# teasgen/speech_separation

Measured on AMD Instinct MI355X. Metric: mixtures/sec (2-spk, 4 s @ 8 kHz) DPTN-AV forward, higher is better.
Workload: dtype f32; 1 GPU; configs[2]: DPTN-AV (dptn_wav_av) forward, precomputed lip embeddings, batch=16 per GPU, T=32000, random-init weights (numpy seed 0); batch_per_gpu=16, samples=32000, parallelism=dp1 (batch shards, no data-path collective)

## Files before the change

### speech_separation_amd/csrc/attn_block.h

```cpp
#pragma once
#include "common.h"

constexpr int ATTN_BLOCK_MAX_LEN = 160;
size_t attn_block_lds_bytes(int nkb);
struct AttnFfnPrologue {
  const float* hc;
  const float* wf;
  const float* bf;
  const float* g2;
  const float* b2;
};
constexpr int ATTN_PACK_IN = 3 * 128 * 128, ATTN_PACK_OUT = 128 * 128, ATTN_PACK_FFN = 128 * 256;
constexpr int ATTN_PACK_FLOATS = ATTN_PACK_IN + ATTN_PACK_OUT + ATTN_PACK_FFN;
struct AttnPackSrc {
  const float* w_in;
  const float* w_o;
  const float* w_f;
};
constexpr int ATTN_PACK_MAX_PATHS = 32;
int attn_pack_launch(void* stream, const AttnPackSrc* src, int npaths, float* dst );
int attn_block_launch(void* stream, const float* x, const float* w_in, const float* b_in, const float* w_o, const float* b_o,
                      const float* gamma, const float* beta, float* y1, const SeqGeom& g, bool split = false,
                      const AttnFfnPrologue* pro = nullptr, const float* wpack = nullptr);

size_t attn_block2_lds_bytes(int nkb, bool pro);
int attn_block2_launch(void* stream, const float* x, const float* b_in, const float* b_o, const float* gamma, const float* beta,
                       float* y1, const SeqGeom& g, const AttnFfnPrologue* pro, const float* wpack);
```

### speech_separation_amd/csrc/attn_block2.hip

```cpp
#include <hip/hip_runtime.h>

#include "attn_block.h"
#include "vmem_asm.h"

namespace {

constexpr int N = 128, DH = 32;
constexpr int LDX = N + 4;
constexpr int LDHC = 256 + 4;
constexpr int OB_FLOATS = 4 * 4 * 64 * 4;

constexpr int kb_mfmas(int kb, int nkb) { return (kb > 0 ? 16 : 0) + (kb + 1 < nkb ? 16 : 0); }

DEV void ln_group_stats(f32x16& v, float& mu_w, float& m2_w) {
  f32x2 s0 = (f32x2){v[0], v[1]} + (f32x2){v[2], v[3]}, s1 = (f32x2){v[4], v[5]} + (f32x2){v[6], v[7]};
  s0 += (f32x2){v[8], v[9]};
  s1 += (f32x2){v[10], v[11]};
  s0 += (f32x2){v[12], v[13]};
  s1 += (f32x2){v[14], v[15]};
  const f32x2 s = s0 + s1;
  mu_w = half_sum(s.x + s.y) * (1.0f / 32);
  const f32x2 m2 = (f32x2){mu_w, mu_w};
  f32x2 q0 = (f32x2){0.f, 0.f}, q1 = (f32x2){0.f, 0.f};
#pragma unroll
  for (int r = 0; r < 16; r += 4) {
    const f32x2 d0 = (f32x2){v[r], v[r + 1]} - m2, d1 = (f32x2){v[r + 2], v[r + 3]} - m2;
    v[r] = d0.x; v[r + 1] = d0.y; v[r + 2] = d1.x; v[r + 3] = d1.y;
    q0 += d0 * d0;
    q1 += d1 * d1;
  }
  const f32x2 q = q0 + q1;
  m2_w = half_sum(q.x + q.y);
}
DEV float ln_merge(const float4 a, const float4 b, float mu_w, float& delta) {
  const float mu = ((a.x + a.z) + (b.x + b.z)) * 0.25f;
  const float d0 = a.x - mu, d1 = a.z - mu, d2 = b.x - mu, d3 = b.z - mu;
  const float m2 = ((a.y + a.w) + (b.y + b.w)) + 32.0f * ((d0 * d0 + d1 * d1) + (d2 * d2 + d3 * d3));
  delta = mu_w - mu;
  return rsqrtf(m2 * (1.0f / N) + 1e-5f);
}

struct FfnPro2 {
  const float* hc;
  const float* wf;
  const float* bf;
  const float* g2;
  const float* b2;
};

#ifdef ATTN_STAMPS
__device__ unsigned long long g_ab2_stamps[16];
DEV unsigned long long ab_now() {
  unsigned long long t;
  asm volatile("s_memtime %0\n\ts_waitcnt lgkmcnt(0)" : "=s"(t) :: "memory");
  return t;
}
#define AB_DECL unsigned long long ab_t[12] = {0, 0, 0, 0, 0, 0, 0, 0, 0, 0, 0, 0}; unsigned long long ab_last = ab_now();
#define AB_MARK(i) { const unsigned long long ab_n = ab_now(); ab_t[i] += ab_n - ab_last; ab_last = ab_n; }
#define AB_KEEP(x) asm volatile("" :: "v"(x));
#define AB_END                                                                                      \
  if ((threadIdx.x & 63) == 0) {                                                                    \
    for (int ab_i = 0; ab_i < 12; ++ab_i) atomicAdd(&g_ab2_stamps[ab_i], ab_t[ab_i]);               \
    atomicAdd(&g_ab2_stamps[12], 1ull);                                                             \
  }
#else
#define AB_DECL
#define AB_MARK(i)
#define AB_KEEP(x)
#define AB_END
#endif

template <int NKB, bool PRO>
__global__ __launch_bounds__(256) void attn_block2_kernel(const float* __restrict__ x, const float* __restrict__ wp_in,
                                                          const float* __restrict__ b_in, const float* __restrict__ wp_o,
                                                          const float* __restrict__ b_o, const float* __restrict__ gamma,
                                                          const float* __restrict__ beta, float* __restrict__ y1, SeqGeom g,
                                                          float scale_log2e, FfnPro2 pro) {
  extern __shared__ __attribute__((aligned(16))) float smem[];
  float* Xs = smem;
  float* Hs = smem + NKB * 32 * LDX;
  float* Ob = Hs;
  float* Red = Hs + (PRO ? 2 * 32 * LDHC : OB_FLOATS);
  float* Cst = Red + 512;
  const int tid = threadIdx.x;
  const int h = __builtin_amdgcn_readfirstlane(tid >> 6);
  const int lane = tid & 63, c = lane & 31, hh = lane >> 5;
  const int seq = blockIdx.x, len = g.len;
  const int64_t tok0 = seq_token_base(g, seq);
  const int tstride = seq_token_stride(g);
  const unsigned rs_y = (unsigned)tstride * 512u;
  char* const ybase = reinterpret_cast<char*>(y1) + tok0 * 512;
  auto row_off = [&](int row, unsigned rstride, bool clamp) -> unsigned {
    if (clamp) row = row < len ? row : len - 1;
    return (unsigned)__umul24((unsigned)row, rstride);
  };
  const unsigned frag_col = (unsigned)(32 * h + 4 * hh);

  AB_DECL
  if (tid < (PRO ? 192 : 96)) {
    const int which = tid >> 5, q4 = tid & 31;
    const float* src = which == 0 ? b_o : which == 1 ? gamma : which == 2 ? beta : which == 3 ? pro.bf : which == 4 ? pro.g2 : pro.b2;
    *reinterpret_cast<float4*>(&Cst[which * 128 + 4 * q4]) = ldg4(src + 4 * q4);
  }
  auto cst16 = [&](int which, f32x16& d) {
#pragma unroll
    for (int j = 0; j < 4; ++j) {
      const float4 t = *reinterpret_cast<const float4*>(&Cst[which * 128 + frag_col + 8 * j]);
      d[4 * j + 0] = t.x; d[4 * j + 1] = t.y; d[4 * j + 2] = t.z; d[4 * j + 3] = t.w;
    }
  };
  auto red_put = [&](int par, float mu_w, float m2_w) {
    *reinterpret_cast<float2*>(&Red[par * 256 + (c * 4 + h) * 2]) = make_float2(mu_w, m2_w);
  };
  auto red_get = [&](int par, float mu_w, float& delta) {
    const float4 a = *reinterpret_cast<const float4*>(&Red[par * 256 + c * 8]), b = *reinterpret_cast<const float4*>(&Red[par * 256 + c * 8 + 4]);
    return ln_merge(a, b, mu_w, delta);
  };

  float wkf[64], wvf[64];
  auto fetch_wkv1 = [&](int m) {
    const float* wk = wp_in + ((1 * 4 + h) * 16 * 64 + lane) * 4;
    const float* wv = wp_in + ((2 * 4 + h) * 16 * 64 + lane) * 4;
    const float4 a = ldg4(wk + m * 256), b = ldg4(wv + m * 256);
    wkf[4 * m + 0] = a.x; wkf[4 * m + 1] = a.y; wkf[4 * m + 2] = a.z; wkf[4 * m + 3] = a.w;
    wvf[4 * m + 0] = b.x; wvf[4 * m + 1] = b.y; wvf[4 * m + 2] = b.z; wvf[4 * m + 3] = b.w;
  };
  auto fetch_wkv = [&]() {
#pragma unroll
    for (int m = 0; m < 16; ++m) fetch_wkv1(m);
  };
  if constexpr (PRO) {
    f32x4 wf4[32];
    const uint32_t lane16 = (uint32_t)lane * 16u;
    {
      const char* wb = reinterpret_cast<const char*>(pro.wf + h * 32 * 64 * 4);
      static_for<8>([&](auto MQ) {
        constexpr int mq = decltype(MQ)::value;
        ldg4_uncounted_a<0>(wf4[4 * mq + 0], wb + mq * 4096, lane16);
        ldg4_uncounted_a<1024>(wf4[4 * mq + 1], wb + mq * 4096, lane16);
        ldg4_uncounted_a<2048>(wf4[4 * mq + 2], wb + mq * 4096, lane16);
        ldg4_uncounted_a<3072>(wf4[4 * mq + 3], wb + mq * 4096, lane16);
      });
    }
    const uint32_t hs_lds = lds_addr(Hs);
    const char* const hbase = reinterpret_cast<const char*>(pro.hc) + tok0 * 1024;
    const uint32_t rs_h = (uint32_t)tstride * 1024u;
    constexpr bool TRI = NKB >= 4;
    auto hbuf_lds = [&](int b) -> uint32_t {
      if (TRI) return (b % 3) == 2 ? lds_addr(Xs) + (uint32_t)((NKB - 2) * 32 * LDX * 4) : hs_lds + (uint32_t)((b % 3) * 32 * LDHC * 4);
      return hs_lds + (uint32_t)((b & 1) * 32 * LDHC * 4);
    };
    auto hbuf = [&](int b) -> const float* { return TRI ? ((b % 3) == 2 ? Xs + (NKB - 2) * 32 * LDX : Hs + (b % 3) * 32 * LDHC) : Hs + (b & 1) * 32 * LDHC; };
    f32x4 res[2][4];
    auto issue_d1 = [&](auto RB, int i) {
      constexpr int rb = decltype(RB)::value;
      int row = rb * 32 + 8 * h + i;
      if (rb == NKB - 1) row = row < len ? row : len - 1;
      dma_part<false>(hbase + (uint32_t)row * rs_h, lane16, hbuf_lds(rb) + (uint32_t)((8 * h + i) * LDHC * 4));
    };
    auto issue_r1 = [&](auto RB, f32x4 (&rr)[4], int j) {
      constexpr int rb = decltype(RB)::value;
      const unsigned ro = row_off(rb * 32 + c, rs_y, rb == NKB - 1) + 4u * frag_col;
      switch (j) {
        case 0: ldg4_uncounted<0>(rr[0], ybase, ro); break;
        case 1: ldg4_uncounted<32>(rr[1], ybase, ro); break;
        case 2: ldg4_uncounted<64>(rr[2], ybase, ro); break;
        default: ldg4_uncounted<96>(rr[3], ybase, ro); break;
      }
    };
    auto issue_d = [&](auto RB) {
#pragma unroll
      for (int i = 0; i < 8; ++i) issue_d1(RB, i);
    };
    auto issue_r = [&](auto RB, f32x4 (&rr)[4]) {
#pragma unroll
      for (int j = 0; j < 4; ++j) issue_r1(RB, rr, j);
    };
    constexpr int AHEAD = TRI ? 2 : 1;
    issue_d(std::integral_constant<int, 0>{});
    issue_r(std::integral_constant<int, 0>{}, res[0]);
    constexpr int BEHIND_WF = 12;
    wait_vm_a16<BEHIND_WF>(wf4);
    wait_vm_a16<BEHIND_WF>(wf4 + 16);
    AB_MARK(0)
    f32x16 vprev = zero16();
    float mu_prev = 0.f;
    auto normalise_prev = [&](int pb) {
      float delta;
      const float rstd = red_get(pb & 1, mu_prev, delta);
      f32x16 g2c, b2c;
      cst16(4, g2c);
      cst16(5, b2c);
      const f32x2 d2 = (f32x2){delta, delta}, r2 = (f32x2){rstd, rstd};
      float* xw = &Xs[(pb * 32 + c) * LDX + frag_col];
#pragma unroll
      for (int j = 0; j < 4; ++j) {
        const f32x2 lo = ((f32x2){vprev[4 * j], vprev[4 * j + 1]} + d2) * r2 * (f32x2){g2c[4 * j], g2c[4 * j + 1]} + (f32x2){b2c[4 * j], b2c[4 * j + 1]};
        const f32x2 hi = ((f32x2){vprev[4 * j + 2], vprev[4 * j + 3]} + d2) * r2 * (f32x2){g2c[4 * j + 2], g2c[4 * j + 3]} +
                         (f32x2){b2c[4 * j + 2], b2c[4 * j + 3]};
        *reinterpret_cast<float4*>(xw + 8 * j) = make_float4(lo.x, lo.y, hi.x, hi.y);
      }
    };
    auto pro_block = [&](auto RB) {
      constexpr int rb = decltype(RB)::value;
      constexpr int KEEP = (AHEAD == 2 && rb >= 1 && rb + 1 < NKB) ? 8 : 0;
      wait_vm<KEEP>(res[rb & 1]);
      __syncthreads();
      AB_MARK(1)
      constexpr bool HAS_R = rb + 1 < NKB, HAS_D = rb + AHEAD < NKB && rb + AHEAD >= 2, HAS_D1 = rb == 0 && NKB > 1;
      constexpr int NREQ = rb == NKB - 1 ? 16 : 4 + (HAS_D1 ? 8 : 0) + (HAS_D ? 8 : 0);
      auto request = [&](int k) {
        if constexpr (rb == NKB - 1) {
          fetch_wkv1(k);
        } else if (k < 4) {
          if constexpr (HAS_R) issue_r1(std::integral_constant<int, HAS_R ? rb + 1 : 0>{}, res[(rb + 1) & 1], k);
        } else if (HAS_D1 && k < 12) {
          if constexpr (HAS_D1) issue_d1(std::integral_constant<int, 1>{}, k - 4);
        } else {
          if constexpr (HAS_D) issue_d1(std::integral_constant<int, HAS_D ? rb + AHEAD : 0>{}, k - (HAS_D1 ? 12 : 4));
        }
      };
      f32x16 a0 = zero16(), a1 = zero16();
      const float* ar = hbuf(rb) + c * LDHC + 4 * hh;
#pragma unroll
      for (int m0 = 0; m0 < 32; m0 += 8) {
        float4 af[8];
#pragma unroll
        for (int m = 0; m < 8; ++m) af[m] = *reinterpret_cast<const float4*>(ar + 8 * (m0 + m));
#pragma unroll
        for (int m = 0; m < 8; ++m) {
          a0 = mfma32(wf4[m0 + m][0], af[m].x, a0);
          a1 = mfma32(wf4[m0 + m][1], af[m].y, a1);
          a0 = mfma32(wf4[m0 + m][2], af[m].z, a0);
          a1 = mfma32(wf4[m0 + m][3], af[m].w, a1);
          constexpr int EVERY = NREQ > 12 ? 1 : 2;
          if ((m0 + m) % EVERY == EVERY - 1 && (m0 + m) / EVERY < NREQ && (m0 + m) < 24) {
            __builtin_amdgcn_sched_barrier(0);
            request((m0 + m) / EVERY);
            __builtin_amdgcn_sched_barrier(0);
          }
        }
// ... 9 lines not shown
      AB_KEEP(a0[15]) AB_KEEP(a1[15])
      AB_MARK(2)
      f32x16 bfc;
      cst16(3, bfc);
#pragma unroll
      for (int r = 0; r < 16; r += 2) {
        const f32x2 t = ((f32x2){a0[r], a0[r + 1]} + (f32x2){a1[r], a1[r + 1]}) + (f32x2){bfc[r], bfc[r + 1]} +
                        (f32x2){res[rb & 1][r >> 2][r & 3], res[rb & 1][r >> 2][(r & 3) + 1]};
        vprev[r] = t.x;
        vprev[r + 1] = t.y;
      }
      float m2_w;
      ln_group_stats(vprev, mu_prev, m2_w);
      red_put(rb & 1, mu_prev, m2_w);
      AB_MARK(3)
    };
    static_for<NKB>(pro_block);
    __syncthreads();
    normalise_prev(NKB - 1);
    AB_MARK(4)
  } else {
    constexpr int NLD = NKB * 4;
    float4 st[NLD];
#pragma unroll
    for (int i = 0; i < NLD; ++i) {
      const int row = i * 8 + (tid >> 5);
      st[i] = *reinterpret_cast<const float4*>(reinterpret_cast<const char*>(x) + tok0 * 512 + row_off(row, rs_y, i >= 4 * (NKB - 1)) +
                                               16u * (tid & 31));
    }
    fetch_wkv();
#pragma unroll
    for (int i = 0; i < NLD; ++i) *reinterpret_cast<float4*>(&Xs[(i * 8 + (tid >> 5)) * LDX + 4 * (tid & 31)]) = st[i];
  }
  __syncthreads();
  AB_MARK(5)

  float wqf[64];
  {
    const float* wq = wp_in + ((0 * 4 + h) * 16 * 64 + lane) * 4;
#pragma unroll
    for (int m = 0; m < 16; ++m) {
      const float4 a = ldg4(wq + m * 256);
      wqf[4 * m + 0] = a.x; wqf[4 * m + 1] = a.y; wqf[4 * m + 2] = a.z; wqf[4 * m + 3] = a.w;
    }
  }
  f32x16 kt[NKB], vv[NKB];
  {
    const float bv = b_in[2 * N + h * DH + c];
    float bk[16];
#pragma unroll
    for (int j = 0; j < 4; ++j) {
      const float4 t = ldg4(b_in + N + h * DH + 8 * j + 4 * hh);
      bk[4 * j + 0] = t.x; bk[4 * j + 1] = t.y; bk[4 * j + 2] = t.z; bk[4 * j + 3] = t.w;
    }
#pragma unroll
    for (int rb = 0; rb < NKB; ++rb) {
      const float* xr = &Xs[(rb * 32 + c) * LDX + 4 * hh];
      f32x16 ka = zero16(), va = zero16();
#pragma unroll
      for (int m0 = 0; m0 < 16; m0 += 8) {
        float4 xf[8];
#pragma unroll
        for (int m = 0; m < 8; ++m) xf[m] = *reinterpret_cast<const float4*>(xr + 8 * (m0 + m));
#pragma unroll
        for (int m = 0; m < 8; ++m) {
          const float xa[4] = {xf[m].x, xf[m].y, xf[m].z, xf[m].w};
#pragma unroll
          for (int t = 0; t < 4; ++t) {
            ka = mfma32(wkf[4 * (m0 + m) + t], xa[t], ka);
            va = mfma32(xa[t], wvf[4 * (m0 + m) + t], va);
          }
        }
      }
#pragma unroll
      for (int r = 0; r < 16; r += 2) {
        const f32x2 tk = (f32x2){ka[r], ka[r + 1]} + (f32x2){bk[r], bk[r + 1]}, tv = (f32x2){va[r], va[r + 1]} + (f32x2){bv, bv};
        kt[rb][r] = tk.x; kt[rb][r + 1] = tk.y;
        vv[rb][r] = tv.x; vv[rb][r + 1] = tv.y;
      }
#pragma unroll
      for (int r = 0; r < 16; ++r) asm volatile("" : "+a"(kt[rb][r]), "+a"(vv[rb][r]));
      __builtin_amdgcn_sched_barrier(0);
    }
  }

  AB_MARK(6)
#pragma unroll
  for (int i = 0; i < 64; ++i) asm volatile("" : "+a"(wqf[i]));
  float wo2[4][16];
#pragma unroll
  for (int hp = 0; hp < 4; ++hp) {
    const float* wr = wp_o + (((hp * 4 + h) * 4) * 64 + lane) * 4;
#pragma unroll
    for (int j = 0; j < 4; ++j) {
      const float4 t = ldg4(wr + j * 256);
      wo2[hp][4 * j + 0] = t.x; wo2[hp][4 * j + 1] = t.y; wo2[hp][4 * j + 2] = t.z; wo2[hp][4 * j + 3] = t.w;
    }
  }
  float qbias[16];
#pragma unroll
  for (int j = 0; j < 4; ++j) {
    const float4 t = ldg4(b_in + h * DH + 8 * j + 4 * hh);
    qbias[4 * j + 0] = t.x; qbias[4 * j + 1] = t.y; qbias[4 * j + 2] = t.z; qbias[4 * j + 3] = t.w;
  }

  auto q_tile_mfmas = [&](int qb, f32x16& q0, f32x16& q1) {
    const float* xr = &Xs[(qb * 32 + c) * LDX + 4 * hh];
#pragma unroll
    for (int m0 = 0; m0 < 16; m0 += 8) {
      float4 xf[8];
#pragma unroll
      for (int m = 0; m < 8; ++m) xf[m] = *reinterpret_cast<const float4*>(xr + 8 * (m0 + m));
#pragma unroll
      for (int m = 0; m < 8; ++m) {
        q0 = mfma32(wqf[4 * (m0 + m) + 0], xf[m].x, q0);
        q1 = mfma32(wqf[4 * (m0 + m) + 1], xf[m].y, q1);
// ... 140 lines not shown
    AB_MARK(9)
    __builtin_amdgcn_sched_barrier(0);
    if (qb + 1 < NKB) {
      qa = zero16();
      qb_ = zero16();
      q_tile_mfmas(qb + 1, qa, qb_);
    }
    {
      const float rstd = red_get(0, mu_w, delta);
      f32x16 gac, bec;
      cst16(1, gac);
      cst16(2, bec);
      const f32x2 d2 = (f32x2){delta, delta}, r2 = (f32x2){rstd, rstd};
      char* yw = ybase + row_off(qb * 32 + c, rs_y, true) + 4u * frag_col;
#pragma unroll
      for (int j = 0; j < 4; ++j) {
        const f32x2 lo = ((f32x2){v[4 * j], v[4 * j + 1]} + d2) * r2 * (f32x2){gac[4 * j], gac[4 * j + 1]} + (f32x2){bec[4 * j], bec[4 * j + 1]};
        const f32x2 hi = ((f32x2){v[4 * j + 2], v[4 * j + 3]} + d2) * r2 * (f32x2){gac[4 * j + 2], gac[4 * j + 3]} +
                         (f32x2){bec[4 * j + 2], bec[4 * j + 3]};
        *reinterpret_cast<float4*>(yw + 32 * j) = make_float4(lo.x, lo.y, hi.x, hi.y);
      }
    }
    if (qb + 1 < NKB) {
#pragma unroll
      for (int i = 0; i < 64; ++i) {
        __builtin_amdgcn_sched_group_barrier(0x008, 1, 0);
        __builtin_amdgcn_sched_group_barrier(0x1f6, 2, 0);
      }
    }
    __builtin_amdgcn_sched_barrier(0);
    AB_KEEP(qa[15]) AB_KEEP(qb_[15])
    AB_MARK(10)
  }
  AB_END
}

}

size_t attn_block2_lds_bytes(int nkb, bool pro) {
  return sizeof(float) * ((size_t)nkb * 32 * LDX + (pro ? 2 * 32 * LDHC : OB_FLOATS) + 512 + 6 * 128);
}

int attn_block2_launch(void* stream, const float* x, const float* b_in, const float* b_o, const float* gamma, const float* beta,
                       float* y1, const SeqGeom& g, const AttnFfnPrologue* pro, const float* wpack) {
  using Kern = void (*)(const float*, const float*, const float*, const float*, const float*, const float*, const float*, float*,
                        SeqGeom, float, FfnPro2);
  const int nkb = (g.len + 31) / 32;
  if (nkb < 1 || nkb > 5 || !wpack) return (int)hipErrorInvalidValue;
  const float scale_log2e = 1.4426950408889634f / sqrtf((float)DH);
  const int dev = current_hip_device();
  Kern kern;
  const bool p = pro != nullptr;
  switch (nkb) {
    case 1: kern = p ? attn_block2_kernel<1, true> : attn_block2_kernel<1, false>; break;
    case 2: kern = p ? attn_block2_kernel<2, true> : attn_block2_kernel<2, false>; break;
    case 3: kern = p ? attn_block2_kernel<3, true> : attn_block2_kernel<3, false>; break;
    case 4: kern = p ? attn_block2_kernel<4, true> : attn_block2_kernel<4, false>; break;
    default: kern = p ? attn_block2_kernel<5, true> : attn_block2_kernel<5, false>; break;
  }
  const size_t lds = attn_block2_lds_bytes(nkb, p);
  static PerDeviceOnce ready_all[2][6];
  PerDeviceOnce* ready = ready_all[p ? 1 : 0];
  if (!ready[nkb].done(dev)) {
    hipError_t e = hipFuncSetAttribute(reinterpret_cast<const void*>(kern), hipFuncAttributeMaxDynamicSharedMemorySize, (int)lds);
    if (e != hipSuccess) return (int)e;
    ready[nkb].set(dev);
  }
  FfnPro2 fp{};
  if (p) fp = FfnPro2{pro->hc, pro->wf, pro->bf, pro->g2, pro->b2};
  hipLaunchKernelGGL(kern, dim3(g.nseq), dim3(256), lds, static_cast<hipStream_t>(stream), x, wpack, b_in, wpack + ATTN_PACK_IN,
                     b_o, gamma, beta, y1, g, scale_log2e, fp);
  return (int)hipGetLastError();
}

#ifdef ATTN_STAMPS
extern "C" int dptnav_debug_attn2_stamps(unsigned long long* out, int reset) {
  if (reset) {
    unsigned long long z[16] = {0};
    return (int)hipMemcpyToSymbol(HIP_SYMBOL(g_ab2_stamps), z, sizeof(z));
  }
  if (hipDeviceSynchronize() != hipSuccess) return -1;
  return (int)hipMemcpyFromSymbol(out, HIP_SYMBOL(g_ab2_stamps), 16 * sizeof(unsigned long long));
}
#endif
```

### speech_separation_amd/csrc/dptnav.hip

```cpp
#include <hip/hip_runtime.h>

#include <cmath>
#include <cstdarg>
#include <cstdio>
#include <cstring>
#include <string>
#include <vector>

#include "../../include/dptnav.h"
#include "attention.h"
#include "attn_block.h"
#include "attn_block64.h"
#include "common.h"
#include "gemm_ws.h"
#include "headtail.h"
#include "lstm.h"
#include "lstm16.h"
#include "fcln.h"
#include "dgrad_t.h"
#include "dgrad_r.h"
#include "gemm_t.h"
#include "sisnr.h"
#include "train_tail.h"
#include "backward.h"
// ... 44 lines not shown

enum ProfCat { CAT_VIDEO = 0, CAT_ENCODER, CAT_QKV, CAT_ATTN, CAT_OUTPROJ, CAT_LSTM_PRE, CAT_LSTM, CAT_FFN,
               CAT_SEP, CAT_POST, CAT_DECODER, CAT_COUNT };
static const char* const kProfNames[CAT_COUNT] = {
    "video_linear", "encoder_fuse", "qkv_gemm", "attention", "outproj_ln_gemm", "lstm_pre_gemm",
    "lstm_recurrence", "ffn_ln_gemm", "sep_gemm", "postproc_gemm", "decoder_gather"};

struct ProfRec {
  int cat;
  hipEvent_t a, b;
};

struct dptnav_ctx {
  dptnav_config cfg;
  bool prof_on = false;
  bool opt_lstm_stamps = false;
  bool opt_overlap = true;
  bool opt_serialize = false;
  bool opt_lstm16 = true;
  int opt_fuse_pre128 = 1;
  bool fuse128_for(int B) const { return opt_fuse_pre128 == 2 || (opt_fuse_pre128 == 1 && B >= 12); }
  int opt_fcln = 1;
  bool opt_fuse_pre = true;
  bool opt_pack_whh = true;
  bool opt_pack_wih = true;
  bool opt_deterministic = false;
  int opt_lstm4 = 1;
  bool opt_split_bf16 = false;
  bool opt_fuse_attn = true;
  bool opt_gemm_t = true;
  bool opt_dgrad_r = true;
  bool opt_dgrad_t = true;
  bool opt_attn_v2 = true;
  bool opt_fold_tail = true;
  bool opt_wgrad_ride = true;
  bool opt_wgrad2 = true;
  bool opt_ln_tape = true;
  bool opt_fuse_ffn = true;
  int opt_lstm_diag = 0;
  int opt_inject_fail = 0;
  bool opt_debug_sync = false;
  bool opt_train_fuse_probe = false;
  int opt_dropout_ppm = 0;
  unsigned opt_dropout_seed = 0;
  DropCfg drop_cfg(int block, int path, bool train, int half = 0) const {
    DropCfg d{0u, 0u, 1.0f};
    if (!train || opt_dropout_ppm <= 0) return d;
    const double p = opt_dropout_ppm * 1e-6;
    d.seed = opt_dropout_seed ^ (0x9E3779B9u * (unsigned)(2 * block + path + 1)) ^ (0x7F4A7C15u * (unsigned)half);
    d.thresh = (unsigned)(p * 16777216.0);
    d.inv_keep = (float)(1.0 / (1.0 - p));
    return d;
  }
  static constexpr int NSTREAMS = 4;
  hipStream_t streams[NSTREAMS] = {nullptr, nullptr, nullptr, nullptr};
  hipEvent_t ev_fork = nullptr, ev_join[NSTREAMS] = {nullptr, nullptr, nullptr, nullptr}, ev_lstm[2] = {nullptr, nullptr};
  hipEvent_t ev_side[2][4] = {{nullptr, nullptr, nullptr, nullptr}, {nullptr, nullptr, nullptr, nullptr}};
  bool opt_wgrad_side = true;
  int opt_sub_batches = 0;
  int opt_lstm_inflight = 0;
  int opt_split_policy = 1;
  bool opt_lstm_chain = false;
  std::vector<hipEvent_t> ev_sub;
  int ensure_sub_events(int n) {
    while ((int)ev_sub.size() < n) {
      hipEvent_t e = nullptr;
// ... 560 lines not shown
  const int64_t ntiles = (M + BM - 1) / BM;
  const bool dptn = g.arch == 0;
  const float* lstm_in = dptn ? y1 : x_in;

  const bool fused = dptn && (!pb.train || c->opt_train_fuse_probe) && path_fusable<N>(c, path, B, S);
  if (fused && (chain & CHAIN_PRO) && c->pw[2 * block + path - 1].ndir != 2)
    return c->fail(DPTNAV_ERR_INVALID, "internal: FFN prologue needs both LSTM directions of the previous path");
  if (fused && N == 64) {
    ProfScope ps(c, CAT_ATTN, st);
    AttnFfnPrologue pro{};
    if (chain & CHAIN_PRO) {
      const PathWeights& pw = c->pw[2 * block + path - 1];
      pro = AttnFfnPrologue{hc, pw.ffn_w, pw.ffn_b, pw.ln2_w, pw.ln2_b};
    }
    const int rc = attn_block64_launch(st, x_in, w.in_w, w.in_b, w.out_w, w.out_b, w.ln1_w, w.ln1_b, y1, geom,
                                       (chain & CHAIN_PRO) ? &pro : nullptr);
    if (rc != 0) return c->fail(DPTNAV_ERR_HIP, "attention block (N = 64): %s", hipGetErrorString((hipError_t)rc));
  } else if (fused) {
    ProfScope ps(c, CAT_ATTN, st);
    AttnFfnPrologue pro{};
    if (chain & CHAIN_PRO) {
      const PathWeights& pw = c->pw[2 * block + path - 1];
      pro = AttnFfnPrologue{hc, pw.ffn_w, pw.ffn_b, pw.ln2_w, pw.ln2_b};
    }
    const float* wpack = nullptr;
    if (!c->opt_split_bf16) {
      float* pk = ws + pl.wpack + (size_t)(2 * block + path) * ATTN_PACK_FLOATS;
      if (!run.packed) {
        if (int rc = pack_attn_weights(c, st, 2 * block + path, 1, pk)) return rc;
      }
      wpack = pk;
      if (chain & CHAIN_PRO) pro.wf = pk - ATTN_PACK_FLOATS + ATTN_PACK_IN + ATTN_PACK_OUT;
    }
    const int rc = (c->opt_attn_v2 && !c->opt_split_bf16)
                       ? attn_block2_launch(st, x_in, w.in_b, w.out_b, w.ln1_w, w.ln1_b, y1, geom, (chain & CHAIN_PRO) ? &pro : nullptr, wpack)
                       : attn_block_launch(st, x_in, w.in_w, w.in_b, w.out_w, w.out_b, w.ln1_w, w.ln1_b, y1, geom, c->opt_split_bf16,
                                           (chain & CHAIN_PRO) ? &pro : nullptr, wpack);
    if (rc != 0) return c->fail(DPTNAV_ERR_HIP, "attention block: %s", hipGetErrorString((hipError_t)rc));
  } else if (chain & CHAIN_PRO) {
    return c->fail(DPTNAV_ERR_INVALID, "internal: FFN prologue requested for an unfused attention block");
  }
  if (dptn && !fused) {
    int done = 0;
    if constexpr (N == 128) {
      if (pb.train && c->opt_gemm_t) {
        if (int rc = inject_failure(c, "qkv gemm")) return rc;
        if (run.slot + 1 > QUEUE_SLOTS) return c->fail(DPTNAV_ERR_INVALID, "qkv gemm: ticket counters exhausted");
        float* wp = ws + pl.winp + (run.packed_inw ? (size_t)(2 * block + path) * 3 * N * N : 0);
        if (!run.packed_inw)
          if (int rc = pack_inw(c, st, 2 * block + path, 1, wp)) return rc;
        GemmTArgs ga;
        ga.A = x_in; ga.Wpacked = wp; ga.bias = w.in_b; ga.out = qkv; ga.M = M; ga.nout = 3 * N;
        unsigned* const queue = run.take_queue(1);
        ga.queue = c->opt_deterministic ? nullptr : queue;
        ProfScope ps(c, CAT_QKV, st);
        const int rc = gemm_t_launch(st, ga, c->num_cus);
        if (rc == 0) done = 1;
        else if (rc == (int)hipErrorInvalidValue) { (void)hipGetLastError(); run.slot -= 1; }
        else return c->fail(DPTNAV_ERR_HIP, "qkv gemm: %s", hipGetErrorString((hipError_t)rc));
      }
    }
    if (!done) {
      ALoadDense al{x_in, M, N, BM};
      EpiBiasStore ep{qkv, w.in_b, M, 3 * N, BM, 3 * N};
      if (int rc = launch_gemm<N, 3, WR, WC>(c, run, CAT_QKV, "qkv gemm", w.in_w, ntiles, 1, al, ep)) return rc;
    }
  }
  if (dptn && !fused)
// ... 1856 lines not shown
  return DPTNAV_OK;
}

int dptnav_dropout_mask(dptnav_handle h, int block, int path, int B, int S, float* mask, void* stream) {
  if (!h || !mask) return DPTNAV_ERR_INVALID;
  const SeqGeom geom = make_geom(path, B, S, h->cfg.chunk_size);
  hipLaunchKernelGGL(dropout_mask_kernel, dim3(geom.nseq, h->cfg.num_heads), dim3(256), 0, (hipStream_t)stream, mask, geom,
                     h->cfg.num_heads, h->drop_cfg(block, path, true));
  LAUNCH_CHECK(h, "dropout mask");
  return DPTNAV_OK;
}

int dptnav_set_option(dptnav_handle h, const char* key, int value) {
  if (!h || !key) return DPTNAV_ERR_INVALID;
  const std::string k(key);
  if (k == "lstm_stamps") h->opt_lstm_stamps = value != 0;
  else if (k == "dropout_ppm" && value >= 0 && value < 1000000) h->opt_dropout_ppm = value;
  else if (k == "dropout_seed") h->opt_dropout_seed = (unsigned)value;
  else if (k == "overlap") h->opt_overlap = value != 0;
  else if (k == "serialize") h->opt_serialize = value != 0;
  else if (k == "deterministic") h->opt_deterministic = value != 0;
  else if (k == "pack_wih") h->opt_pack_wih = value != 0;
  else if (k == "fuse_pre") h->opt_fuse_pre = value != 0;
  else if (k == "fcln" && value >= 0 && value <= 2) h->opt_fcln = value;
  else if (k == "fuse_pre128" && value >= 0 && value <= 2) h->opt_fuse_pre128 = value;
  else if (k == "pack_whh") h->opt_pack_whh = value != 0;
  else if (k == "lstm16") h->opt_lstm16 = value != 0;
  else if (k == "lstm4") {
    if (value < 0 || value > 2) return h->fail(DPTNAV_ERR_INVALID, "lstm4: 0, 1 or 2");
    h->opt_lstm4 = (int)value;
  }
  else if (k == "fuse_attn") h->opt_fuse_attn = value != 0;
  else if (k == "attn_v2") h->opt_attn_v2 = value != 0;
  else if (k == "dgrad_t") h->opt_dgrad_t = value != 0;
  else if (k == "dgrad_r") h->opt_dgrad_r = value != 0;
  else if (k == "gemm_t") h->opt_gemm_t = value != 0;
  else if (k == "fuse_ffn") h->opt_fuse_ffn = value != 0;
  else if (k == "wgrad2") h->opt_wgrad2 = value != 0;
  else if (k == "ln_tape") h->opt_ln_tape = value != 0;
  else if (k == "fold_tail") h->opt_fold_tail = value != 0;
  else if (k == "wgrad_ride") h->opt_wgrad_ride = value != 0;
  else if (k == "wgrad_side") h->opt_wgrad_side = value != 0;
  else if (k == "sub_batches" && value >= 0 && value <= MAX_SUB) h->opt_sub_batches = value;
  else if (k == "lstm_inflight" && value >= 0 && value <= MAX_SUB) h->opt_lstm_inflight = value;
  else if (k == "split_policy" && (value == 0 || value == 1)) h->opt_split_policy = value;
  else if (k == "lstm_chain") h->opt_lstm_chain = value != 0;
  else if (k == "split_bf16") h->opt_split_bf16 = value != 0;
  else if (k == "train_overlap") h->opt_train_overlap = value != 0;
  else if (k == "lstm_diag") h->opt_lstm_diag = (int)value;
  else if (k == "inject_fail") h->opt_inject_fail = value;
  else if (k == "debug_sync") h->opt_debug_sync = value != 0;
  else if (k == "train_fuse_probe") h->opt_train_fuse_probe = value != 0;
  else return h->fail(DPTNAV_ERR_INVALID, "unknown option '%s'", key);
  return DPTNAV_OK;
}

int dptnav_profile_enable(dptnav_handle h, int on) {
  if (!h) return DPTNAV_ERR_INVALID;
  h->prof_on = on != 0;
  return DPTNAV_OK;
}
int dptnav_profile_collect(dptnav_handle h) {
  if (!h) return DPTNAV_ERR_INVALID;
  for (ProfRec& r : h->prof_pending) {
    float ms = 0.f;
    hipError_t e = hipEventSynchronize(r.b);
// ... 50 lines not shown
```

### speech_separation_amd/csrc/vmem_asm.h

```cpp
#pragma once
#include "common.h"

DEV uint32_t lds_addr(const void* p) { return (uint32_t)(uintptr_t)(const __attribute__((address_space(3))) void*)p; }

template <bool HALF>
DEV void dma_part(const void* sbase, uint32_t voff, uint32_t lds_base) {
  if constexpr (!HALF) {
    asm volatile("s_mov_b32 m0, %0\n\ts_nop 4\n\tglobal_load_lds_dwordx4 %1, %2" ::"s"(lds_base), "v"(voff), "s"(sbase) : "memory", "m0");
  } else {
    uint32_t saved;
    asm volatile("s_mov_b32 m0, %1\n\ts_mov_b32 %0, exec_hi\n\ts_mov_b32 exec_hi, 0\n\ts_nop 4\n\tglobal_load_lds_dwordx4 %2, %3\n\ts_mov_b32 exec_hi, %0"
                 : "=&s"(saved)
                 : "s"(lds_base), "v"(voff), "s"(sbase)
                 : "memory", "m0");
  }
}
DEV void dma16(const void* g, uint32_t lds_base) {
  asm volatile("s_mov_b32 m0, %0\n\ts_nop 0\n\tglobal_load_lds_dwordx4 %1, off" ::"s"(lds_base), "v"(g) : "memory", "m0");
}

template <int OFF>
DEV void ldg4_uncounted(f32x4& dst, const void* sbase, uint32_t voff) {
  asm volatile("s_nop 4\n\tglobal_load_dwordx4 %0, %1, %2 offset:%3" : "=v"(dst) : "v"(voff), "s"(sbase), "n"(OFF) : "memory");
}
// ... 11 lines not shown
  asm volatile("s_waitcnt vmcnt(%[n])" : "+v"(r[0]), "+v"(r[1]), "+v"(r[2]), "+v"(r[3]) : [n] "n"(KEEP) : "memory");
}
template <int KEEP>
DEV void wait_vm_v16(f32x4* r) {
  asm volatile("s_waitcnt vmcnt(%[n])"
               : "+v"(r[0]), "+v"(r[1]), "+v"(r[2]), "+v"(r[3]), "+v"(r[4]), "+v"(r[5]), "+v"(r[6]), "+v"(r[7]), "+v"(r[8]), "+v"(r[9]),
                 "+v"(r[10]), "+v"(r[11]), "+v"(r[12]), "+v"(r[13]), "+v"(r[14]), "+v"(r[15])
               : [n] "n"(KEEP)
               : "memory");
}
template <int KEEP>
DEV void wait_vm_a16(f32x4* r) {
  asm volatile("s_waitcnt vmcnt(%[n])"
               : "+a"(r[0]), "+a"(r[1]), "+a"(r[2]), "+a"(r[3]), "+a"(r[4]), "+a"(r[5]), "+a"(r[6]), "+a"(r[7]), "+a"(r[8]), "+a"(r[9]),
                 "+a"(r[10]), "+a"(r[11]), "+a"(r[12]), "+a"(r[13]), "+a"(r[14]), "+a"(r[15])
               : [n] "n"(KEEP)
               : "memory");
}
template <int KEEP>
DEV void wait_vm1(int& r) {
  asm volatile("s_waitcnt vmcnt(%[n])" : "+v"(r) : [n] "n"(KEEP) : "memory");
}
template <int KEEP>
DEV void retire_vm1(int r) {
  asm volatile("s_waitcnt vmcnt(%[n])" ::"v"(r), [n] "n"(KEEP) : "memory");
}

struct TicketLoop {
  int ticket_ahead;
  int* s_next;
  unsigned* queue;
  int ntiles;
  bool dyn;

  DEV TicketLoop(int* s_next_, unsigned* queue_, int ntiles_) : ticket_ahead(0), s_next(s_next_), queue(queue_), ntiles(ntiles_), dyn(queue_ != nullptr) {
    if (dyn) {
      if (threadIdx.x == 0) {
        s_next[0] = (int)atomicAdd(queue, 1u);
        ticket_ahead = (int)atomicAdd(queue, 1u);
      }
    } else if (threadIdx.x == 0) {
      s_next[0] = (int)blockIdx.x;
    }
  }
  DEV int first_tile() const { return __builtin_amdgcn_readfirstlane(s_next[0]); }

  DEV int next_tile(int tile, int buf) {
    const int tid = threadIdx.x;
    if (dyn && tid == 0) s_next[buf ^ 1] = ticket_ahead;
    __syncthreads();
    const int next = dyn ? __builtin_amdgcn_readfirstlane(s_next[buf ^ 1]) : tile + (int)gridDim.x;
    if (dyn && tid == 0)
      asm volatile("s_nop 4\n\tglobal_atomic_add %0, %1, %2, %3 sc0" : "=v"(ticket_ahead) : "v"(0u), "v"(1u), "s"(queue) : "memory");
    return next;
  }
  template <class Body>
  DEV void run(int& tile, int& buf, Body&& body) {
    bool first = true;
    while (true) {
      const int next = next_tile(tile, buf);
      if (next < ntiles) {
        if (first) body(std::true_type{}, std::false_type{}, next);
        else body(std::true_type{}, std::true_type{}, next);
        first = false;
        tile = next;
        buf ^= 1;
      } else {
        if (first) body(std::false_type{}, std::false_type{}, next);
        else body(std::false_type{}, std::true_type{}, next);
        break;
      }
    }
  }
  template <int KEEP>
  DEV void wait() {
    wait_vm1<KEEP>(ticket_ahead);
  }
  template <int KEEP>
  DEV void retire() const {
    retire_vm1<KEEP>(ticket_ahead);
  }
};
// ... 1 lines not shown
```

Measured before the change: 568.6 mixtures/sec.

## Make attention block kernel persistent with ticket queue and cross-sequence prefetch

Turns attn_block2 into a persistent kernel when sequence count exceeds CU count. Workgroups pull the next sequence from an atomic ticket queue. During the current K/V projection they prefetch the next sequence's FFN hidden rows into LDS, and double-buffer swap indices change to match. This is meant to amortize per-block launch and prologue cost and hide the next sequence's load latency. The cost is extra atomics, tighter register and LDS usage, and a harder schedule.

```diff
diff --git a/speech_separation_amd/csrc/attn_block.h b/speech_separation_amd/csrc/attn_block.h
--- a/speech_separation_amd/csrc/attn_block.h
+++ b/speech_separation_amd/csrc/attn_block.h
@@ -25,4 +25,5 @@
 
 size_t attn_block2_lds_bytes(int nkb, bool pro);
 int attn_block2_launch(void* stream, const float* x, const float* b_in, const float* b_o, const float* gamma, const float* beta,
-                       float* y1, const SeqGeom& g, const AttnFfnPrologue* pro, const float* wpack);
+                       float* y1, const SeqGeom& g, const AttnFfnPrologue* pro, const float* wpack, unsigned* queue = nullptr,
+                       int persist_grid = 0);
diff --git a/speech_separation_amd/csrc/attn_block2.hip b/speech_separation_amd/csrc/attn_block2.hip
--- a/speech_separation_amd/csrc/attn_block2.hip
+++ b/speech_separation_amd/csrc/attn_block2.hip
@@ -55,41 +55,56 @@
   asm volatile("s_memtime %0\n\ts_waitcnt lgkmcnt(0)" : "=s"(t) :: "memory");
   return t;
 }
-#define AB_DECL unsigned long long ab_t[12] = {0, 0, 0, 0, 0, 0, 0, 0, 0, 0, 0, 0}; unsigned long long ab_last = ab_now();
+#define AB_DECL unsigned long long ab_t[13] = {0, 0, 0, 0, 0, 0, 0, 0, 0, 0, 0, 0, 0}, ab_seqs = 0; unsigned long long ab_last = ab_now();
+#define AB_SEQ ++ab_seqs;
 #define AB_MARK(i) { const unsigned long long ab_n = ab_now(); ab_t[i] += ab_n - ab_last; ab_last = ab_n; }
 #define AB_KEEP(x) asm volatile("" :: "v"(x));
 #define AB_END                                                                                      \
   if ((threadIdx.x & 63) == 0) {                                                                    \
-    for (int ab_i = 0; ab_i < 12; ++ab_i) atomicAdd(&g_ab2_stamps[ab_i], ab_t[ab_i]);               \
-    atomicAdd(&g_ab2_stamps[12], 1ull);                                                             \
+    for (int ab_i = 0; ab_i < 13; ++ab_i) atomicAdd(&g_ab2_stamps[ab_i], ab_t[ab_i]);               \
+    atomicAdd(&g_ab2_stamps[15], ab_seqs);       \
   }
 #else
 #define AB_DECL
+#define AB_SEQ
 #define AB_MARK(i)
 #define AB_KEEP(x)
 #define AB_END
 #endif
 
-template <int NKB, bool PRO>
-__global__ __launch_bounds__(256) void attn_block2_kernel(const float* __restrict__ x, const float* __restrict__ wp_in,
-                                                          const float* __restrict__ b_in, const float* __restrict__ wp_o,
+struct NoTickets {
+  struct StaticFirst {};
+  DEV NoTickets(int*, unsigned*, int, StaticFirst) {}
+  DEV int next_tile(int, int) {
+    __syncthreads();
+    return 0;
+  }
+  template <int KEEP>
+  DEV void wait() {}
+  template <int KEEP>
+  DEV void retire() const {}
+};
+
+template <int NKB, bool PRO, bool PERSIST>
+__global__ __launch_bounds__(256) void attn_block2_kernel(const float* __restrict__ x_, const float* __restrict__ wp_in_,
+                                                          const float* __restrict__ b_in_, const float* __restrict__ wp_o_,
                                                           const float* __restrict__ b_o, const float* __restrict__ gamma,
-                                                          const float* __restrict__ beta, float* __restrict__ y1, SeqGeom g,
-                                                          float scale_log2e, FfnPro2 pro) {
+                                                          const float* __restrict__ beta, float* __restrict__ y1_, SeqGeom g,
+                                                          float scale_log2e, FfnPro2 pro_, unsigned* queue) {
+  static_assert(PRO || !PERSIST, "the persistent form exists with the FFN prologue only");
   extern __shared__ __attribute__((aligned(16))) float smem[];
   float* Xs = smem;
   float* Hs = smem + NKB * 32 * LDX;
   float* Ob = Hs;
   float* Red = Hs + (PRO ? 2 * 32 * LDHC : OB_FLOATS);
   float* Cst = Red + 512;
+  int* Tks = reinterpret_cast<int*>(Cst + 6 * 128);
   const int tid = threadIdx.x;
   const int h = __builtin_amdgcn_readfirstlane(tid >> 6);
   const int lane = tid & 63, c = lane & 31, hh = lane >> 5;
-  const int seq = blockIdx.x, len = g.len;
-  const int64_t tok0 = seq_token_base(g, seq);
+  const int len = g.len;
   const int tstride = seq_token_stride(g);
   const unsigned rs_y = (unsigned)tstride * 512u;
-  char* const ybase = reinterpret_cast<char*>(y1) + tok0 * 512;
   auto row_off = [&](int row, unsigned rstride, bool clamp) -> unsigned {
     if (clamp) row = row < len ? row : len - 1;
     return (unsigned)__umul24((unsigned)row, rstride);
@@ -99,7 +114,7 @@
   AB_DECL
   if (tid < (PRO ? 192 : 96)) {
     const int which = tid >> 5, q4 = tid & 31;
-    const float* src = which == 0 ? b_o : which == 1 ? gamma : which == 2 ? beta : which == 3 ? pro.bf : which == 4 ? pro.g2 : pro.b2;
+    const float* src = which == 0 ? b_o : which == 1 ? gamma : which == 2 ? beta : which == 3 ? pro_.bf : which == 4 ? pro_.g2 : pro_.b2;
     *reinterpret_cast<float4*>(&Cst[which * 128 + 4 * q4]) = ldg4(src + 4 * q4);
   }
   auto cst16 = [&](int which, f32x16& d) {
@@ -117,6 +132,19 @@
     return ln_merge(a, b, mu_w, delta);
   };
 
+  using Tickets = std::conditional_t<PERSIST, TicketLoop, NoTickets>;
+  Tickets tk(Tks, queue, g.nseq, typename Tickets::StaticFirst{});
+  int seq = blockIdx.x;
+  int tkbuf = 0;
+  bool fetched0 = false;
+  for (;;) {
+  AB_SEQ
+  const float *x = x_, *wp_in = wp_in_, *b_in = b_in_, *wp_o = wp_o_;
+  float* y1 = y1_;
+  FfnPro2 pro = pro_;
+  if constexpr (PERSIST) asm volatile("" : "+s"(x), "+s"(wp_in), "+s"(wp_o), "+s"(y1), "+s"(b_in), "+s"(pro.hc), "+s"(pro.wf));
+  const int64_t tok0 = seq_token_base(g, seq);
+  char* const ybase = reinterpret_cast<char*>(y1) + tok0 * 512;
   float wkf[64], wvf[64];
   auto fetch_wkv1 = [&](int m) {
     const float* wk = wp_in + ((1 * 4 + h) * 16 * 64 + lane) * 4;
@@ -132,6 +160,47 @@
   if constexpr (PRO) {
     f32x4 wf4[32];
     const uint32_t lane16 = (uint32_t)lane * 16u;
+    const uint32_t hs_lds = lds_addr(Hs);
+    const char* const hbase = reinterpret_cast<const char*>(pro.hc) + tok0 * 1024;
+    const uint32_t rs_h = (uint32_t)tstride * 1024u;
+    constexpr bool TRI = NKB >= 4;
+    constexpr int SW = PERSIST ? 1 : 0;
+    auto hbuf_lds = [&](int b) -> uint32_t {
+      if (TRI) return (b % 3) == 2 ? lds_addr(Xs) + (uint32_t)((NKB - 2) * 32 * LDX * 4) : hs_lds + (uint32_t)(((b % 3) ^ SW) * 32 * LDHC * 4);
+      return hs_lds + (uint32_t)(((b & 1) ^ SW) * 32 * LDHC * 4);
+    };
+    auto hbuf = [&](int b) -> const float* {
+      return TRI ? ((b % 3) == 2 ? Xs + (NKB - 2) * 32 * LDX : Hs + ((b % 3) ^ SW) * 32 * LDHC) : Hs + ((b & 1) ^ SW) * 32 * LDHC;
+    };
+    f32x4 res[2][4];
+    auto issue_d1 = [&](auto RB, int i) {
+      constexpr int rb = decltype(RB)::value;
+      int row = rb * 32 + 8 * h + i;
+      if (rb == NKB - 1) row = row < len ? row : len - 1;
+      dma_part<false>(hbase + (uint32_t)row * rs_h, lane16, hbuf_lds(rb) + (uint32_t)((8 * h + i) * LDHC * 4));
+    };
+    auto issue_r1 = [&](auto RB, f32x4 (&rr)[4], int j) {
+      constexpr int rb = decltype(RB)::value;
+      const unsigned ro = row_off(rb * 32 + c, rs_y, rb == NKB - 1) + 4u * frag_col;
+      switch (j) {
+        case 0: ldg4_uncounted<0>(rr[0], ybase, ro); break;
+        case 1: ldg4_uncounted<32>(rr[1], ybase, ro); break;
+        case 2: ldg4_uncounted<64>(rr[2], ybase, ro); break;
+        default: ldg4_uncounted<96>(rr[3], ybase, ro); break;
+      }
+    };
+    auto issue_d = [&](auto RB) {
+#pragma unroll
+      for (int i = 0; i < 8; ++i) issue_d1(RB, i);
+    };
+    auto issue_r = [&](auto RB, f32x4 (&rr)[4]) {
+#pragma unroll
+      for (int j = 0; j < 4; ++j) issue_r1(RB, rr, j);
+    };
+    constexpr int AHEAD = TRI ? 2 : 1;
+    if constexpr (PERSIST) {
+      if (!fetched0) issue_d(std::integral_constant<int, 0>{});
+    }
     {
       const char* wb = reinterpret_cast<const char*>(pro.wf + h * 32 * 64 * 4);
       static_for<8>([&](auto MQ) {
@@ -142,46 +211,12 @@
         ldg4_uncounted_a<3072>(wf4[4 * mq + 3], wb + mq * 4096, lane16);
       });
     }
-    const uint32_t hs_lds = lds_addr(Hs);
-    const char* const hbase = reinterpret_cast<const char*>(pro.hc) + tok0 * 1024;
-    const uint32_t rs_h = (uint32_t)tstride * 1024u;
-    constexpr bool TRI = NKB >= 4;
-    auto hbuf_lds = [&](int b) -> uint32_t {
-      if (TRI) return (b % 3) == 2 ? lds_addr(Xs) + (uint32_t)((NKB - 2) * 32 * LDX * 4) : hs_lds + (uint32_t)((b % 3) * 32 * LDHC * 4);
-      return hs_lds + (uint32_t)((b & 1) * 32 * LDHC * 4);
-    };
-    auto hbuf = [&](int b) -> const float* { return TRI ? ((b % 3) == 2 ? Xs + (NKB - 2) * 32 * LDX : Hs + (b % 3) * 32 * LDHC) : Hs + (b & 1) * 32 * LDHC; };
-    f32x4 res[2][4];
-    auto issue_d1 = [&](auto RB, int i) {
-      constexpr int rb = decltype(RB)::value;
-      int row = rb * 32 + 8 * h + i;
-      if (rb == NKB - 1) row = row < len ? row : len - 1;
-      dma_part<false>(hbase + (uint32_t)row * rs_h, lane16, hbuf_lds(rb) + (uint32_t)((8 * h + i) * LDHC * 4));
-    };
-    auto issue_r1 = [&](auto RB, f32x4 (&rr)[4], int j) {
-      constexpr int rb = decltype(RB)::value;
-      const unsigned ro = row_off(rb * 32 + c, rs_y, rb == NKB - 1) + 4u * frag_col;
-      switch (j) {
-        case 0: ldg4_uncounted<0>(rr[0], ybase, ro); break;
-        case 1: ldg4_uncounted<32>(rr[1], ybase, ro); break;
-        case 2: ldg4_uncounted<64>(rr[2], ybase, ro); break;
-        default: ldg4_uncounted<96>(rr[3], ybase, ro); break;
-      }
-    };
-    auto issue_d = [&](auto RB) {
-#pragma unroll
-      for (int i = 0; i < 8; ++i) issue_d1(RB, i);
-    };
-    auto issue_r = [&](auto RB, f32x4 (&rr)[4]) {
-#pragma unroll
-      for (int j = 0; j < 4; ++j) issue_r1(RB, rr, j);
-    };
-    constexpr int AHEAD = TRI ? 2 : 1;
-    issue_d(std::integral_constant<int, 0>{});
+    if constexpr (!PERSIST) issue_d(std::integral_constant<int, 0>{});
     issue_r(std::integral_constant<int, 0>{}, res[0]);
-    constexpr int BEHIND_WF = 12;
+    constexpr int BEHIND_WF = PERSIST ? 4 : 12;
     wait_vm_a16<BEHIND_WF>(wf4);
     wait_vm_a16<BEHIND_WF>(wf4 + 16);
+    tk.template wait<BEHIND_WF>();
     AB_MARK(0)
     f32x16 vprev = zero16();
     float mu_prev = 0.f;
@@ -206,7 +241,7 @@
       constexpr int KEEP = (AHEAD == 2 && rb >= 1 && rb + 1 < NKB) ? 8 : 0;
       wait_vm<KEEP>(res[rb & 1]);
       __syncthreads();
-      AB_MARK(1)
+      AB_MARK(PERSIST && rb == 0 ? 12 : 1)
       constexpr bool HAS_R = rb + 1 < NKB, HAS_D = rb + AHEAD < NKB && rb + AHEAD >= 2, HAS_D1 = rb == 0 && NKB > 1;
       constexpr int NREQ = rb == NKB - 1 ? 16 : 4 + (HAS_D1 ? 8 : 0) + (HAS_D ? 8 : 0);
       auto request = [&](int k) {
@@ -282,8 +317,9 @@
 #pragma unroll
     for (int i = 0; i < NLD; ++i) *reinterpret_cast<float4*>(&Xs[(i * 8 + (tid >> 5)) * LDX + 4 * (tid & 31)]) = st[i];
   }
-  __syncthreads();
-  AB_MARK(5)
+  const int next = tk.next_tile(seq, tkbuf);
+  const bool has_next = PERSIST && next < g.nseq;
+  AB_MARK(PERSIST ? 11 : 5)
 
   float wqf[64];
   {
@@ -303,8 +339,18 @@
       const float4 t = ldg4(b_in + N + h * DH + 8 * j + 4 * hh);
       bk[4 * j + 0] = t.x; bk[4 * j + 1] = t.y; bk[4 * j + 2] = t.z; bk[4 * j + 3] = t.w;
     }
-#pragma unroll
-    for (int rb = 0; rb < NKB; ++rb) {
+    const char* hnext = nullptr;
+    if constexpr (PERSIST) {
+      if (has_next) hnext = reinterpret_cast<const char*>(pro.hc) + seq_token_base(g, next) * 1024;
+    }
+    auto prefetch1 = [&](int k) {
+      int row = 8 * h + k;
+      if (NKB == 1) row = row < len ? row : len - 1;
+      dma_part<false>(hnext + (uint32_t)row * ((uint32_t)tstride * 1024u), (uint32_t)lane * 16u,
+                      lds_addr(Hs) + (uint32_t)((32 + 8 * h + k) * LDHC * 4));
+    };
+    auto kv_block = [&](auto RB, auto PF) {
+      constexpr int rb = decltype(RB)::value;
       const float* xr = &Xs[(rb * 32 + c) * LDX + 4 * hh];
       f32x16 ka = zero16(), va = zero16();
 #pragma unroll
@@ -320,6 +366,13 @@
             ka = mfma32(wkf[4 * (m0 + m) + t], xa[t], ka);
             va = mfma32(xa[t], wvf[4 * (m0 + m) + t], va);
           }
+          if constexpr (decltype(PF)::value) {
+            if ((m0 + m) & 1) {
+              __builtin_amdgcn_sched_barrier(0);
+              prefetch1((m0 + m) >> 1);
+              __builtin_amdgcn_sched_barrier(0);
+            }
+          }
         }
       }
 #pragma unroll
@@ -331,7 +384,15 @@
 #pragma unroll
       for (int r = 0; r < 16; ++r) asm volatile("" : "+a"(kt[rb][r]), "+a"(vv[rb][r]));
       __builtin_amdgcn_sched_barrier(0);
-    }
+    };
+    static_for<NKB>([&](auto RB) {
+      if constexpr (PERSIST && decltype(RB)::value == 0) {
+        if (has_next) kv_block(RB, std::true_type{});
+        else kv_block(RB, std::false_type{});
+      } else {
+        kv_block(RB, std::false_type{});
+      }
+    });
   }
 
   AB_MARK(6)
@@ -538,35 +599,48 @@
     AB_KEEP(qa[15]) AB_KEEP(qb_[15])
     AB_MARK(10)
   }
+  if constexpr (!PERSIST) {
+    break;
+  } else {
+    if (!has_next) {
+      tk.template retire<0>();
+      break;
+    }
+    seq = next;
+    tkbuf ^= 1;
+    fetched0 = true;
+  }
+  }
   AB_END
 }
 
 }
 
 size_t attn_block2_lds_bytes(int nkb, bool pro) {
-  return sizeof(float) * ((size_t)nkb * 32 * LDX + (pro ? 2 * 32 * LDHC : OB_FLOATS) + 512 + 6 * 128);
+  return sizeof(float) * ((size_t)nkb * 32 * LDX + (pro ? 2 * 32 * LDHC : OB_FLOATS) + 512 + 6 * 128 + 4);
 }
 
 int attn_block2_launch(void* stream, const float* x, const float* b_in, const float* b_o, const float* gamma, const float* beta,
-                       float* y1, const SeqGeom& g, const AttnFfnPrologue* pro, const float* wpack) {
+                       float* y1, const SeqGeom& g, const AttnFfnPrologue* pro, const float* wpack, unsigned* queue, int persist_grid) {
   using Kern = void (*)(const float*, const float*, const float*, const float*, const float*, const float*, const float*, float*,
-                        SeqGeom, float, FfnPro2);
+                        SeqGeom, float, FfnPro2, unsigned*);
   const int nkb = (g.len + 31) / 32;
   if (nkb < 1 || nkb > 5 || !wpack) return (int)hipErrorInvalidValue;
   const float scale_log2e = 1.4426950408889634f / sqrtf((float)DH);
   const int dev = current_hip_device();
   Kern kern;
   const bool p = pro != nullptr;
+  const bool persist = p && queue != nullptr && persist_grid > 0;
   switch (nkb) {
-    case 1: kern = p ? attn_block2_kernel<1, true> : attn_block2_kernel<1, false>; break;
-    case 2: kern = p ? attn_block2_kernel<2, true> : attn_block2_kernel<2, false>; break;
-    case 3: kern = p ? attn_block2_kernel<3, true> : attn_block2_kernel<3, false>; break;
-    case 4: kern = p ? attn_block2_kernel<4, true> : attn_block2_kernel<4, false>; break;
-    default: kern = p ? attn_block2_kernel<5, true> : attn_block2_kernel<5, false>; break;
+    case 1: kern = persist ? attn_block2_kernel<1, true, true> : p ? attn_block2_kernel<1, true, false> : attn_block2_kernel<1, false, false>; break;
+    case 2: kern = persist ? attn_block2_kernel<2, true, true> : p ? attn_block2_kernel<2, true, false> : attn_block2_kernel<2, false, false>; break;
+    case 3: kern = persist ? attn_block2_kernel<3, true, true> : p ? attn_block2_kernel<3, true, false> : attn_block2_kernel<3, false, false>; break;
+    case 4: kern = persist ? attn_block2_kernel<4, true, true> : p ? attn_block2_kernel<4, true, false> : attn_block2_kernel<4, false, false>; break;
+    default: kern = persist ? attn_block2_kernel<5, true, true> : p ? attn_block2_kernel<5, true, false> : attn_block2_kernel<5, false, false>; break;
   }
   const size_t lds = attn_block2_lds_bytes(nkb, p);
-  static PerDeviceOnce ready_all[2][6];
-  PerDeviceOnce* ready = ready_all[p ? 1 : 0];
+  static PerDeviceOnce ready_all[3][6];
+  PerDeviceOnce* ready = ready_all[persist ? 2 : p ? 1 : 0];
   if (!ready[nkb].done(dev)) {
     hipError_t e = hipFuncSetAttribute(reinterpret_cast<const void*>(kern), hipFuncAttributeMaxDynamicSharedMemorySize, (int)lds);
     if (e != hipSuccess) return (int)e;
@@ -574,8 +648,9 @@
   }
   FfnPro2 fp{};
   if (p) fp = FfnPro2{pro->hc, pro->wf, pro->bf, pro->g2, pro->b2};
-  hipLaunchKernelGGL(kern, dim3(g.nseq), dim3(256), lds, static_cast<hipStream_t>(stream), x, wpack, b_in, wpack + ATTN_PACK_IN,
-                     b_o, gamma, beta, y1, g, scale_log2e, fp);
+  const int grid = persist ? (g.nseq < persist_grid ? g.nseq : persist_grid) : g.nseq;
+  hipLaunchKernelGGL(kern, dim3(grid), dim3(256), lds, static_cast<hipStream_t>(stream), x, wpack, b_in, wpack + ATTN_PACK_IN,
+                     b_o, gamma, beta, y1, g, scale_log2e, fp, persist ? queue : nullptr);
   return (int)hipGetLastError();
 }
 
diff --git a/speech_separation_amd/csrc/dptnav.hip b/speech_separation_amd/csrc/dptnav.hip
--- a/speech_separation_amd/csrc/dptnav.hip
+++ b/speech_separation_amd/csrc/dptnav.hip
@@ -100,6 +100,7 @@
   bool opt_dgrad_r = true;
   bool opt_dgrad_t = true;
   bool opt_attn_v2 = true;
+  int opt_attn_persist = 1;
   bool opt_fold_tail = true;
   bool opt_wgrad_ride = true;
   bool opt_wgrad2 = true;
@@ -726,8 +727,14 @@
       wpack = pk;
       if (chain & CHAIN_PRO) pro.wf = pk - ATTN_PACK_FLOATS + ATTN_PACK_IN + ATTN_PACK_OUT;
     }
+    unsigned* seq_queue = nullptr;
+    if (c->opt_attn_v2 && !c->opt_split_bf16 && (chain & CHAIN_PRO) && (c->opt_attn_persist > 1 || (c->opt_attn_persist == 1 && geom.nseq > c->num_cus))) {
+      if (run.slot + 1 > QUEUE_SLOTS) return c->fail(DPTNAV_ERR_INVALID, "attention block: ticket counters exhausted");
+      seq_queue = run.take_queue(1);
+    }
     const int rc = (c->opt_attn_v2 && !c->opt_split_bf16)
-                       ? attn_block2_launch(st, x_in, w.in_b, w.out_b, w.ln1_w, w.ln1_b, y1, geom, (chain & CHAIN_PRO) ? &pro : nullptr, wpack)
+                       ? attn_block2_launch(st, x_in, w.in_b, w.out_b, w.ln1_w, w.ln1_b, y1, geom, (chain & CHAIN_PRO) ? &pro : nullptr, wpack, seq_queue,
+                                            c->opt_attn_persist == 1 ? c->num_cus : c->opt_attn_persist)
                        : attn_block_launch(st, x_in, w.in_w, w.in_b, w.out_w, w.out_b, w.ln1_w, w.ln1_b, y1, geom, c->opt_split_bf16,
                                            (chain & CHAIN_PRO) ? &pro : nullptr, wpack);
     if (rc != 0) return c->fail(DPTNAV_ERR_HIP, "attention block: %s", hipGetErrorString((hipError_t)rc));
@@ -2650,6 +2657,7 @@
   }
   else if (k == "fuse_attn") h->opt_fuse_attn = value != 0;
   else if (k == "attn_v2") h->opt_attn_v2 = value != 0;
+  else if (k == "attn_persist" && value >= 0) h->opt_attn_persist = value;
   else if (k == "dgrad_t") h->opt_dgrad_t = value != 0;
   else if (k == "dgrad_r") h->opt_dgrad_r = value != 0;
   else if (k == "gemm_t") h->opt_gemm_t = value != 0;
diff --git a/speech_separation_amd/csrc/vmem_asm.h b/speech_separation_amd/csrc/vmem_asm.h
--- a/speech_separation_amd/csrc/vmem_asm.h
+++ b/speech_separation_amd/csrc/vmem_asm.h
@@ -67,8 +67,9 @@
   unsigned* queue;
   int ntiles;
   bool dyn;
+  int base;
 
-  DEV TicketLoop(int* s_next_, unsigned* queue_, int ntiles_) : ticket_ahead(0), s_next(s_next_), queue(queue_), ntiles(ntiles_), dyn(queue_ != nullptr) {
+  DEV TicketLoop(int* s_next_, unsigned* queue_, int ntiles_) : ticket_ahead(0), s_next(s_next_), queue(queue_), ntiles(ntiles_), dyn(queue_ != nullptr), base(0) {
     if (dyn) {
       if (threadIdx.x == 0) {
         s_next[0] = (int)atomicAdd(queue, 1u);
@@ -78,11 +79,19 @@
       s_next[0] = (int)blockIdx.x;
     }
   }
+  struct StaticFirst {};
+  DEV TicketLoop(int* s_next_, unsigned* queue_, int ntiles_, StaticFirst)
+      : ticket_ahead(0), s_next(s_next_), queue(queue_), ntiles(ntiles_), dyn(queue_ != nullptr), base(queue_ != nullptr ? (int)gridDim.x : 0) {
+    if (threadIdx.x == 0) {
+      s_next[0] = (int)blockIdx.x;
+      if (dyn) asm volatile("s_nop 4\n\tglobal_atomic_add %0, %1, %2, %3 sc0" : "=v"(ticket_ahead) : "v"(0u), "v"(1u), "s"(queue) : "memory");
+    }
+  }
   DEV int first_tile() const { return __builtin_amdgcn_readfirstlane(s_next[0]); }
 
   DEV int next_tile(int tile, int buf) {
     const int tid = threadIdx.x;
-    if (dyn && tid == 0) s_next[buf ^ 1] = ticket_ahead;
+    if (dyn && tid == 0) s_next[buf ^ 1] = ticket_ahead + base;
     __syncthreads();
     const int next = dyn ? __builtin_amdgcn_readfirstlane(s_next[buf ^ 1]) : tile + (int)gridDim.x;
     if (dyn && tid == 0)
```

Result: faster. 576.9 mixtures/sec (median of 6 runs) (+1.5%).
